# PieSil/CUDA-spectral-ray-tracer

Hardware: AMD Instinct MI355X
Metric: Mray/s (higher is better)
Workload: dtype f32; 1 GPU; random-spheres tri scene (4802 tris, 9603 BVH nodes), 1920x1080, 1024 spp, depth 16; scene_id=100, tiles=8x8 px per wave, rank = tile % n_gpus, gather=none (1 GPU), launch_mode=one process, one GPU

## Files before the change

### cuda-spectral-ray-tracer_amd/csrc/srt_device.h

```cpp
#pragma once
#include <hip/hip_runtime.h>
#include <stdint.h>

#include "srt_color_consts.h"
#include "srt_powf.h"

namespace srt {

constexpr int kCieSamples = 95;
constexpr int kWavelengths = 7;
constexpr float kLambdaMin = 360.0f;
constexpr float kLambdaMax = 830.0f;
constexpr float kEpsilon = 0.0001f;
constexpr float kFltMax = 3.402823466e+38f;

__device__ __noinline__ static float dev_powf(float x, float y) { return srt_powf(x, y); }

struct V3 { float x, y, z; };
__device__ __forceinline__ V3 mk(float x, float y, float z) { V3 r; r.x = x; r.y = y; r.z = z; return r; }
__device__ __forceinline__ V3 operator+(V3 a, V3 b) { return mk(a.x + b.x, a.y + b.y, a.z + b.z); }
__device__ __forceinline__ V3 operator-(V3 a, V3 b) { return mk(a.x - b.x, a.y - b.y, a.z - b.z); }
__device__ __forceinline__ V3 operator-(V3 a) { return mk(-a.x, -a.y, -a.z); }
__device__ __forceinline__ V3 operator*(float t, V3 v) { return mk(t * v.x, t * v.y, t * v.z); }
__device__ __forceinline__ float dot(V3 a, V3 b) { return a.x * b.x + a.y * b.y + a.z * b.z; }
// ... 535 lines not shown
        "v_cmpx_gt_u32 vcc, %[ninner], %[node]\n\t"
        SRT_INNER_VISIT_ASM SRT_INNER_NEXT_ASM
        SRT_INNER_VISIT_ASM SRT_INNER_NEXT_ASM
        SRT_INNER_VISIT_ASM SRT_INNER_NEXT_ASM
        SRT_INNER_VISIT_ASM SRT_INNER_NEXT_ASM
        SRT_INNER_VISIT_ASM SRT_INNER_NEXT_ASM
        SRT_INNER_VISIT_ASM SRT_INNER_NEXT_ASM
        SRT_INNER_VISIT_ASM SRT_INNER_NEXT_ASM
        SRT_INNER_VISIT_ASM
        ".Lsrt_burst_end%=:\n\t"
        "s_mov_b64 exec, s[80:81]\n\t"
        : [node] "+v"(tv.node), [top] "+v"(tv.top), [sp] "+v"(tv.sp)
        : [nf0] "v"(tv.nf[0]), [nf1] "v"(tv.nf[1]), [nf2] "v"(tv.nf[2]), [p0] "v"(p0), [p1] "v"(p1), [p2] "v"(p2), [c] "v"(tv.c),
          [ms] "v"(minus_stride), [ps] "v"(plus_stride), [ninner] "s"(n_inner), [refs] "s"(refs), [stay] "s"(stay)
        : "v100", "v101", "v102", "v103", "v104", "v105", "v106", "v107", "v108", "v109", "v110", "v111", "v112", "v113", "v114",
          "v115", "v116", "v117", "v118", "s80", "s81", "s82", "s83", "s84", "s85", "s86", "vcc", "scc", "memory");
}

#define SRT_INNER_NEXT2_ASM                                                                                              \
    "v_cmpx_gt_u32 vcc, %[ninner], %[node]\n\t"                                                                          \
    "s_bcnt1_i32_b64 s86, exec\n\t"                                                                                      \
    "s_cmp_lt_u32 s86, s87\n\t"                                                                                          \
    "s_cbranch_scc1 .Lsrt_phase_burst_end%=\n\t"
__device__ __forceinline__ uint32_t inner_phase_asm(Trav &tv, const NodeSrc &ns, V3 o, V3 inv, uint32_t n_inner, uint32_t n_alive,
                                                    uint32_t score_shade, uint32_t score_fringe) {
    const f2 p0 = mk2(o.x, o.y), p1 = mk2(o.z, inv.x), p2 = mk2(inv.y, inv.z);
    const int minus_stride = -kStackStride<true>, plus_stride = kStackStride<true>;
    const uint32_t refs = (uint32_t)(uintptr_t)ns.lds_r0;
    uint32_t kind;
    asm volatile(
        "s_mov_b64 s[80:81], exec\n\t"
        ".Lsrt_phase_decide%=:\n\t"
        "v_cmp_lt_i32 vcc, -1, %[node]\n\t"
        "v_cmp_le_i32_e64 s[82:83], %[ninner], %[node]\n\t"
        "s_bcnt1_i32_b64 s86, vcc\n\t"
        "s_bcnt1_i32_b64 s87, s[82:83]\n\t"
        "s_sub_u32 s88, %[nalive], s86\n\t"
        "s_sub_u32 s86, s86, s87\n\t"
        "s_mul_i32 s88, s88, %[wshade]\n\t"
        "s_mul_i32 s89, s87, %[wfringe]\n\t"
        "s_lshl_b32 s84, s86, 8\n\t"
        "s_max_u32 s85, s89, s84\n\t"
        "s_mov_b32 %[kind], 0\n\t"
        "s_cmp_gt_u32 s88, s85\n\t"
        "s_cbranch_scc1 .Lsrt_phase_end%=\n\t"
        "s_mov_b32 %[kind], 1\n\t"
        "s_cmp_gt_u32 s89, s84\n\t"
        "s_cbranch_scc1 .Lsrt_phase_end%=\n\t"
        "s_add_u32 s87, s86, 2\n\t"
        "s_mul_hi_u32 s87, s87, 0xaaaaaaab\n\t"
        "s_lshr_b32 s87, s87, 1\n\t"
        "s_andn2_b64 exec, vcc, s[82:83]\n\t"
        SRT_INNER_VISIT_ASM SRT_INNER_NEXT2_ASM
        SRT_INNER_VISIT_ASM SRT_INNER_NEXT2_ASM
        SRT_INNER_VISIT_ASM SRT_INNER_NEXT2_ASM
        SRT_INNER_VISIT_ASM SRT_INNER_NEXT2_ASM
        SRT_INNER_VISIT_ASM SRT_INNER_NEXT2_ASM
        SRT_INNER_VISIT_ASM SRT_INNER_NEXT2_ASM
        SRT_INNER_VISIT_ASM SRT_INNER_NEXT2_ASM
        SRT_INNER_VISIT_ASM
        ".Lsrt_phase_burst_end%=:\n\t"
        "s_mov_b64 exec, s[80:81]\n\t"
        "s_branch .Lsrt_phase_decide%=\n\t"
        ".Lsrt_phase_end%=:\n\t"
        : [node] "+v"(tv.node), [top] "+v"(tv.top), [sp] "+v"(tv.sp), [kind] "=&s"(kind)
        : [nf0] "v"(tv.nf[0]), [nf1] "v"(tv.nf[1]), [nf2] "v"(tv.nf[2]), [p0] "v"(p0), [p1] "v"(p1), [p2] "v"(p2), [c] "v"(tv.c),
          [ms] "v"(minus_stride), [ps] "v"(plus_stride), [ninner] "s"(n_inner), [refs] "s"(refs), [nalive] "s"(n_alive),
          [wshade] "s"(score_shade), [wfringe] "s"(score_fringe)
        : "v100", "v101", "v102", "v103", "v104", "v105", "v106", "v107", "v108", "v109", "v110", "v111", "v112", "v113", "v114",
          "v115", "v116", "v117", "v118", "s80", "s81", "s82", "s83", "s84", "s85", "s86", "s87", "s88", "s89", "vcc",
          "scc", "memory");
    return kind;
}

#define SRT_INNER_VISIT_MIXED_ASM                                                                                        \
    "ds_write_b32 %[sp], %[top] offset:256\n\t"                                                                          \
    "ds_read_b32 v116, %[sp]\n\t"                                                                              \
    "v_cmp_le_u32 vcc, %[ncached], %[node]\n\t"                                          \
    "s_and_saveexec_b64 s[90:91], vcc\n\t"                                                                               \
    "s_cbranch_execz 1f\n\t"                                                                                             \
    "v_mul_u32_u24 v117, 0x50, %[node]\n\t"                                                          \
    "v_add_u32 v114, v117, %[g0]\n\t"                                                                                    \
    "v_add_u32 v115, v117, %[g1]\n\t"                                                                                    \
    "v_add_u32 v118, v117, %[g2]\n\t"                                                                                    \
    "buffer_load_dwordx4 v[100:103], v114, %[rsrc], 0 offen\n\t"                                                         \
    "buffer_load_dwordx4 v[104:107], v115, %[rsrc], 0 offen offset:24\n\t"                                               \
// ... 61 lines not shown
__device__ __forceinline__ void inner_burst4_mixed_asm(Trav &tv, const NodeSrc &ns, V3 o, V3 inv, uint32_t n_inner, uint32_t stay) {
    const f2 p0 = mk2(o.x, o.y), p1 = mk2(o.z, inv.x), p2 = mk2(inv.y, inv.z);
    const int minus_stride = -kStackStride<false>, plus_stride = kStackStride<false>;
    const uint32_t refs0 = (uint32_t)(uintptr_t)ns.lds_r0, refs1 = (uint32_t)(uintptr_t)ns.lds_r1;
    const uint32_t g0 = tv.nf[0] & 8u, g1 = tv.nf[1] & 8u, g2 = tv.nf[2] & 8u;
    asm volatile(
        "s_mov_b64 s[80:81], exec\n\t"
        "v_cmpx_gt_u32 vcc, %[ninner], %[node]\n\t"
        SRT_INNER_VISIT_MIXED_ASM SRT_INNER_NEXT_MIXED_ASM
        SRT_INNER_VISIT_MIXED_ASM SRT_INNER_NEXT_MIXED_ASM
        SRT_INNER_VISIT_MIXED_ASM SRT_INNER_NEXT_MIXED_ASM
        SRT_INNER_VISIT_MIXED_ASM
        ".Lsrt_mixed_end%=:\n\t"
        "s_mov_b64 exec, s[80:81]\n\t"
        : [node] "+v"(tv.node), [top] "+v"(tv.top), [sp] "+v"(tv.sp)
        : [nf0] "v"(tv.nf[0]), [nf1] "v"(tv.nf[1]), [nf2] "v"(tv.nf[2]), [g0] "v"(g0), [g1] "v"(g1), [g2] "v"(g2), [p0] "v"(p0), [p1] "v"(p1), [p2] "v"(p2),
          [c] "v"(tv.c), [ms] "v"(minus_stride), [ps] "v"(plus_stride), [ninner] "s"(n_inner), [ncached] "s"((uint32_t)ns.n_cached), [refs0] "s"(refs0),
          [refs1] "s"(refs1), [stay] "s"(stay), [rsrc] "s"(ns.global_nodes_sw)
        : "v100", "v101", "v102", "v103", "v104", "v105", "v106", "v107", "v108", "v109", "v110", "v111", "v112", "v113", "v114",
          "v115", "v116", "v117", "v118", "s80", "s81", "s82", "s83", "s84", "s85", "s86", "s90", "s91", "vcc", "scc", "memory");
}

struct FringeFetch { f4v q0, q1, q2, q3, q4, q5; int below; };
template <bool NARROW>
__device__ __forceinline__ void trav_fringe_fetch(FringeFetch &ff, const Trav &tv, const NodeSrc &ns, const StackRef &stack) {
    const uint32_t off = __umul24((uint32_t)(tv.node - ns.n_inner), ns.fringe_stride);
    ff.q0 = buf_load16(ns.global_fringe, off); ff.q1 = buf_load16(ns.global_fringe, off + 16u); ff.q2 = buf_load16(ns.global_fringe, off + 32u);
    ff.q3 = buf_load16(ns.global_fringe, off + 48u); ff.q4 = buf_load16(ns.global_fringe, off + 64u); ff.q5 = buf_load16(ns.global_fringe, off + 80u);
    ff.below = NARROW ? (int)*(lds_i16 *)(uintptr_t)tv.sp : *(lds_i32 *)(uintptr_t)tv.sp;
}
template <bool COUNT, bool NARROW, bool PAIRED = false>
__device__ __forceinline__ void trav_fringe_compute(const FringeFetch &ff, Trav &tv, V3 o, V3 d, V3 inv, float tmin, TravStats &ts) {
    const f4v q0 = ff.q0, q1 = ff.q1, q2 = ff.q2, q3 = ff.q3, q4 = ff.q4, q5 = ff.q5;
    const int below = ff.below;
    const f2 w0 = mk2(q0.x, q0.y), w1 = mk2(q0.z, q0.w), w2 = mk2(q1.x, q1.y), w3 = mk2(q1.z, q1.w), w4 = mk2(q2.x, q2.y), w5 = mk2(q2.z, q2.w);
    const f2 w6 = mk2(q3.x, q3.y), w7 = mk2(q3.z, q3.w), w8 = mk2(q4.x, q4.y), w9 = mk2(q4.z, q4.w);
    const uint32_t fl = __float_as_uint(q5.x), fr = __float_as_uint(q5.y);
    const int lref = (int)__float_as_uint(q5.z), rref = (int)__float_as_uint(q5.w);
    const bool leaf_l = PAIRED || lref < 0, leaf_r = PAIRED || rref < 0;
    if (COUNT) { ts.n_iters++; ts.n_tri += (leaf_l ? 1u : 0u) + (leaf_r ? 1u : 0u); ts.n_box += (leaf_l ? 0u : 1u) + (leaf_r ? 0u : 1u); }

    float e_box = 0.f, m_box = 0.f;
    if (!PAIRED) {
        const bool int_r = !leaf_r;
        const float xlo = int_r ? w0.y : w0.x, xhi = int_r ? w1.y : w1.x, ylo = int_r ? w2.y : w2.x, yhi = int_r ? w3.y : w3.x;
        const float zlo = int_r ? w4.y : w4.x, zhi = int_r ? w5.y : w5.x;
        const bool px = inv.x >= 0, py = inv.y >= 0, pz = inv.z >= 0;
        const float t0x = ((px ? xlo : xhi) - o.x) * inv.x, t1x = ((px ? xhi : xlo) - o.x) * inv.x;
        const float t0y = ((py ? ylo : yhi) - o.y) * inv.y, t1y = ((py ? yhi : ylo) - o.y) * inv.y;
        const float t0z = ((pz ? zlo : zhi) - o.z) * inv.z, t1z = ((pz ? zhi : zlo) - o.z) * inv.z;
        e_box = fmaxf(fmaxf(fmaxf(tmin, t0x), t0y), t0z);
        m_box = fminf(fminf(t1x, t1y), t1z);
    }

    const f2 denom = w0 * d.x + w1 * d.y + w2 * d.z;
    const f2 num = w3 - (w0 * o.x + w1 * o.y + w2 * o.z);
    const f2 t = mk2(num.x / denom.x, num.y / denom.y);
    const bool wyl = fl & kTriWIsY, hzl = fl & kTriHIsZ, wyr = fr & kTriWIsY, hzr = fr & kTriHIsZ;
    const f2 pw = mk2(wyl ? o.y : o.x, wyr ? o.y : o.x) + t * mk2(wyl ? d.y : d.x, wyr ? d.y : d.x);
    const f2 ph = mk2(hzl ? o.z : o.y, hzr ? o.z : o.y) + t * mk2(hzl ? d.z : d.y, hzr ? d.z : d.y);
    const f2 a1 = (pw - w6) * (w5 - w7) - (w4 - w6) * (ph - w7);
    const f2 a2 = (pw - w8) * (w7 - w9) - (w6 - w8) * (ph - w9);
    const f2 a3 = (pw - w4) * (w9 - w5) - (w8 - w4) * (ph - w5);
    const uint32_t sl = fl & 0x80000000u, sr = fr & 0x80000000u;
    float m_l = inside_min2(a1.x, a2.x, sl);
    float m_r = inside_min2(a1.y, a2.y, sr);
    asm volatile("" : "+v"(m_l), "+v"(m_r));
    const bool in_l = inside_min3(m_l, a3.x, sl);
    const bool in_r = inside_min3(m_r, a3.y, sr);
    const bool ok_l = leaf_l & !(fabsf(denom.x) < 1e-8f) & (tmin <= t.x) & in_l;
    const bool ok_r = leaf_r & !(fabsf(denom.y) < 1e-8f) & (tmin <= t.y) & in_r;

    const float c0 = tv.c;
    const bool hit_l = ok_l & (t.x <= c0);
    const float c1 = hit_l ? t.x : c0;
    const bool hit_r = ok_r & (t.y <= c1);
    const float c2 = hit_r ? t.y : c1;
    tv.c = c2;
    tv.hit = hit_r ? ~rref : (hit_l ? ~lref : tv.hit);
    const int top = tv.top;
    if (PAIRED) {
        tv.node = top;
        tv.top = below;
        tv.sp += (uint32_t)(-kStackStride<NARROW>);
        return;
    }
    const bool pass = !(fminf(leaf_r ? c0 : c1, m_box) <= e_box);
    const bool go = !(leaf_l & leaf_r) & pass;
    tv.node = go ? (leaf_r ? lref : rref) : top;
    tv.top = go ? top : below;
    tv.sp += (uint32_t)(go ? 0 : -kStackStride<NARROW>);
}
template <bool COUNT, bool NARROW, bool PAIRED = false>
__device__ __forceinline__ void trav_step_fringe(Trav &tv, const NodeSrc &ns, V3 o, V3 d, V3 inv, float tmin, const StackRef &stack, TravStats &ts) {
    FringeFetch ff;
    trav_fringe_fetch<NARROW>(ff, tv, ns, stack);
    trav_fringe_compute<COUNT, NARROW, PAIRED>(ff, tv, o, d, inv, tmin, ts);
}


}
```

### cuda-spectral-ray-tracer_amd/csrc/srt_kernels.hip

```cpp
#include <algorithm>
#include <stdlib.h>

#include "srt_color_consts.h"
#include "srt_kernel_common.h"

namespace srt {

#ifndef SRT_INNER_BURST
#define SRT_INNER_BURST 8
#endif
#ifndef SRT_BURST_DROP
#define SRT_BURST_DROP 3
#endif
#ifndef SRT_ASM_BURST
#define SRT_ASM_BURST 2
#endif
#ifndef SRT_INNER_BURST_L2
#define SRT_INNER_BURST_L2 4
#endif
#ifndef SRT_ASM_BURST_L2
#define SRT_ASM_BURST_L2 1
#endif
#ifndef SRT_BURST_DROP_L2
#define SRT_BURST_DROP_L2 2
// ... 26 lines not shown
}
void render_launch_plan(int stack_depth, int n_records, int n_inner, const PlanKnobs &k, LaunchPlan &lp) {
    render_launch_shape(stack_depth, n_records, n_inner, k, lp.waves_per_block, lp.n_cached);
    lp.all_cached = lp.n_cached == n_inner;
    lp.waves_per_eu = 4;
    lp.blocks_per_cu = 16 / lp.waves_per_block;
    lp.waves_per_cu = lp.waves_per_block * lp.blocks_per_cu;
}
RenderGrid render_launch_grid(const LaunchPlan &lp, uint32_t n_cu, uint32_t waves_per_cu_override, uint32_t queue_rows_bound) {
    RenderGrid g;
    g.waves_per_block = lp.waves_per_block;
    uint32_t waves_per_cu = (uint32_t)lp.waves_per_cu;
    if (waves_per_cu_override > 0 && waves_per_cu_override < 16 && g.waves_per_block == 16) {
        g.waves_per_block = (int)waves_per_cu_override;
        waves_per_cu = waves_per_cu_override;
    }
    uint32_t n_waves = n_cu * waves_per_cu;
    if (n_waves > queue_rows_bound) n_waves = queue_rows_bound;
    g.n_blocks = (n_waves + (uint32_t)g.waves_per_block - 1) / (uint32_t)g.waves_per_block;
    g.waves = g.n_blocks * (uint32_t)g.waves_per_block;
    return g;
}

#ifndef SRT_PAIRED_VARIANT
#define SRT_PAIRED_VARIANT 1
#endif
bool render_paired_variant(bool tree_is_paired, bool narrow, bool all_cached) { return SRT_PAIRED_VARIANT != 0 && tree_is_paired && narrow == all_cached; }

#ifndef SRT_ASSIGN_PERM
#define SRT_ASSIGN_PERM 0
#endif
__device__ __forceinline__ uint32_t assigned_band(uint32_t w) {
    if (SRT_ASSIGN_PERM == 1) return (w & 3u) * 4u + (w >> 2);
    if (SRT_ASSIGN_PERM == 2) return (w & 4u) ? ((w & ~3u) | (3u - (w & 3u))) : w;
    return w;
}

__global__ void init_rng_kernel(uint32_t *rng, uint32_t n_lanes, uint64_t seed) {
    uint32_t idx = blockIdx.x * blockDim.x + threadIdx.x;
    if (idx >= n_lanes) return;
    Rng s;
    rng_seed(s, seed + idx);
    rng[0 * (size_t)n_lanes + idx] = s.d;
    rng[1 * (size_t)n_lanes + idx] = s.v0;
    rng[2 * (size_t)n_lanes + idx] = s.v1;
    rng[3 * (size_t)n_lanes + idx] = s.v2;
// ... 100 lines not shown
    ns.lds_r0 = (lds_cu32 *)s_r0; ns.lds_r1 = (lds_cu32 *)s_r1;
    ns.n_cached = P.n_cached;
    const buf_rsrc shade_rsrc = make_rsrc(P.shade, P.n_tris * 48u);
    const buf_rsrc sd_rsrc = make_rsrc(P.mat_sd, (P.n_materials + 1u) * 768u);
    const uint32_t spp = P.spp;
    uint32_t w_shade = P.score_shade, w_fringe = P.score_fringe;
    asm volatile("" : "+s"(w_shade), "+s"(w_fringe));
    StackRef my_stack;
    {
        const size_t slots = (size_t)(P.stack_depth < 1 ? 1 : P.stack_depth) + kStackSentinels;
        my_stack.s16 = (lds_i16 *)(s_stack_base + (size_t)wave * slots * 128u) + lane;
        my_stack.s32 = (lds_i32 *)(s_stack_base + (size_t)wave * slots * 256u) + lane;
        stack_init<NARROW>(my_stack);
    }

    bool dead = false, have_path = false, have_pixel = false;
    uint32_t idx = 0;
    uint32_t out_slot = 0;
    uint32_t pixel_ij = 0;
    Rng rs; rs.d = rs.v0 = rs.v1 = rs.v2 = rs.v3 = rs.v4 = 0u;
    V3 acc = mk(0.f, 0.f, 0.f);
    float acc2 = 0.f;
    uint32_t sample = 0, bounce = 0, valid = 0;
    V3 ro = mk(0.f, 0.f, 0.f), rd = mk(0.f, 0.f, 1.f), inv = mk(0.f, 0.f, 1.f);
    float hero = kLambdaMin;
    float pw[kWavelengths];
#pragma unroll
    for (int k = 0; k < kWavelengths; k++) pw[k] = 0.f;
    Trav tv; tv.node = kTravIdle; tv.sp = 0u; tv.top = -1; tv.c = kFltMax; tv.hit = -1; tv.nf[0] = tv.nf[1] = tv.nf[2] = 0u;
    uint32_t n_rays = 0;
    TravStats ts;
    bool parked = false, exclusive = false;
    OrderProfile prof;
    prof.magic = 0; prof.seg = nullptr;
    if (COUNT && P.wave_debug) prof = *reinterpret_cast<const OrderProfile *>(P.wave_debug);
    unsigned long long t_shade = 0, t_inner = 0, t_fringe = 0, t_mark = 0;
    if (COUNT) t_mark = __builtin_amdgcn_s_memtime();
    const unsigned long long t_born = t_mark;
    unsigned long long t_dry = 0;
    uint32_t cur_tile_local = 0, pixel_iters0 = 0;
    uint32_t pixel_rays0 = 0, max_pix_iters = 0, max_pix_rays = 0;
    uint32_t w_shade_passes = 0, l_shade = 0, l_cam = 0, w_reject_iters = 0;
    uint32_t n_hits = 0;

    for (;;) {
        if (__ballot(have_pixel) == 0ull) parked = false;
        if (__ballot(!dead && !parked && tv.node < 0) != 0ull) {
            bool end_path = false, begin_trav = false;
            if (COUNT) { w_shade_passes++; l_shade += (uint32_t)__popcll(__ballot(!dead && tv.node == kTravDone)); }
            float xyz_x = 0.0f, xyz_y = 0.0f, xyz_z = 0.0f;

            if (!dead && tv.node == kTravDone) {
                tv.node = kTravIdle;
                if (COUNT && P.wave_debug && prof.seg != nullptr) {
                    const bool walked = !(rd.x != rd.x || rd.y != rd.y || rd.z != rd.z);
                    const unsigned long long m = __ballot(walked);
                    if (walked) {
                        const int leader = __ffsll((long long)m) - 1;
                        uint32_t base = 0;
                        if ((int)lane == leader) base = atomicAdd(prof.seg_tickets, (uint32_t)__popcll(m));
                        base = (uint32_t)__shfl((int)base, leader, 64);
                        const uint32_t ticket = base + (uint32_t)__popcll(m & ((1ull << lane) - 1ull));
                        const uint32_t key = ticket + prof.seg_phase;
                        const uint32_t slot = key / prof.seg_stride - (prof.seg_phase ? 1u : 0u);
                        if (key % prof.seg_stride == 0u && (unsigned long long)slot < prof.seg_capacity) {
                            const float t_end = tv.hit < 0 ? kFltMax : tv.c;
                            prof.seg[2 * (size_t)slot] = make_float4(ro.x, ro.y, ro.z, rd.x);
                            prof.seg[2 * (size_t)slot + 1] = make_float4(rd.y, rd.z, t_end, __int_as_float(tv.hit));
                        }
                    }
                }
                float wl[kWavelengths];
                hero_expand(hero, wl);
                uint32_t sd_table = P.n_materials;
                bool was_hit = false, hit_scattered = false;
                if (tv.hit < 0) {
                    end_path = true;
                } else {
                    if (COUNT && P.wave_debug && prof.magic == kOrderProfileMagic) {
                        int k = prof.leaf[tv.hit];
                        for (int guard = 0; guard < 96; guard++) {
                            const int up = prof.up[k];
                            if (up < 0) break;
                            const float *b = prof.sibbox + 6 * (size_t)k;
                            const float x0 = (b[0] - ro.x) * inv.x, x1 = (b[1] - ro.x) * inv.x;
                            const float y0 = (b[2] - ro.y) * inv.y, y1 = (b[3] - ro.y) * inv.y;
                            const float z0 = (b[4] - ro.z) * inv.z, z1 = (b[5] - ro.z) * inv.z;
                            const float e = fmaxf(fmaxf(fmaxf(0.0f, fminf(x0, x1)), fminf(y0, y1)), fminf(z0, z1));
                            const float m = fminf(fminf(fmaxf(x0, x1), fmaxf(y0, y1)), fmaxf(z0, z1));
                            if (e <= m && e > tv.c) atomicAdd(&prof.cnt[up], 1u);
                            k = up >> 1;
                        }
                    }
                    const uint32_t srec = __umul24((uint32_t)tv.hit, 48u);
                    const f4v s0 = buf_load16(shade_rsrc, srec), s1 = buf_load16(shade_rsrc, srec + 16u), s2 = buf_load16(shade_rsrc, srec + 32u);
                    const V3 n_geo = mk(s0.x, s0.y, s0.z);
                    const V3 hp = ro + tv.c * rd;
                    const bool front_face = dot(rd, n_geo) < 0;
                    const V3 n = front_face ? n_geo : -n_geo;
                    const uint32_t mat = __float_as_uint(s0.w);
                    const uint32_t mtype = __float_as_uint(s1.x);
                    const float fuzz = s1.y;

                    V3 scatter_direction = mk(0.f, 0.f, 0.f);
                    float eps_sign = 1.0f;
                    bool did_scatter = true;
                    const V3 unit_in = unit_vector(rd);
                    if (mtype == 4u) {
                        did_scatter = false;
                    } else if (mtype == 2u) {
                        float ir = sellmeier_index(s1.z, s1.w, s2.x, s2.y, s2.z, s2.w, wl[0]);
                        float refraction_ratio = front_face ? (1.0f / ir) : ir;
                        float cos_theta = fminf(dot(-unit_in, n), 1.0f);
                        float sin_theta = sqrtf(1.0f - cos_theta * cos_theta);
                        bool cannot_refract = refraction_ratio * sin_theta > 1.0f;
                        if (!cannot_refract)
                            cannot_refract = reflectance(cos_theta, refraction_ratio) > rng_uniform(rs);
                        if (cannot_refract) {
                            scatter_direction = reflect(unit_in, n);
                        } else {
                            scatter_direction = refract(unit_in, n, refraction_ratio);
                            eps_sign = -1.0f;
                            valid = 1;
                        }
                    } else {
                        const V3 ruv = random_unit_vector(rs);
                        if (mtype == 1u) {
                            V3 reflected = reflect(unit_in, n);
                            scatter_direction = reflected + fuzz * ruv;
                            did_scatter = dot(scatter_direction, n) > 0;
// ... 1 lines not shown
                        } else {
                            scatter_direction = n + ruv;
                            if (near_zero(scatter_direction)) scatter_direction = n;
                        }
                    }
                    if constexpr (FEATURES) {
                        if (bounce == 0u) {
                            const uint32_t rows_lo = (uint32_t)__builtin_amdgcn_readfirstlane((int)((FILM && !ADAPT) ? U->accum_sum2[0] : U->accum_film[0])), rows_hi = (uint32_t)__builtin_amdgcn_readfirstlane((int)((FILM && !ADAPT) ? U->accum_sum2[1] : U->accum_film[1]));
                            const uint32_t col_lo = (uint32_t)__builtin_amdgcn_readfirstlane((int)((ADAPT || FILM) ? U->tile_cost[0] : U->accum_sum2[0])), col_hi = (uint32_t)__builtin_amdgcn_readfirstlane((int)((ADAPT || FILM) ? U->tile_cost[1] : U->accum_sum2[1]));
                            float4 *row = join_ptr<float4>(rows_lo, rows_hi) + (size_t)idx * (kFeatureStride / 4u);
                            if constexpr (FILM && ADAPT) row += (size_t)U->n_lanes * (kFilmStride / 4u);
                            const buf_rsrc col_rsrc = make_rsrc(join_ptr<const float>(col_lo, col_hi), P.n_materials * 16u);
                            const uint32_t col_off = (mat < P.n_materials ? mat : P.n_materials) * 16u;
                            {
                                float4 f = row[0];
                                const float red = __uint_as_float(__builtin_amdgcn_raw_buffer_load_b32(col_rsrc, (int)col_off, 0, 0));
                                f.x = f.x + n.x; f.y = f.y + n.y; f.z = f.z + n.z; f.w = f.w + red;
                                row[0] = f;
                            }
                            asm volatile("" ::: "memory");
                            {
                                float4 f = row[1];
                                const float2 gb = buf_load8(col_rsrc, col_off + 4u);
                                const float dist = tv.c * sqrtf((rd.x * rd.x + rd.y * rd.y) + rd.z * rd.z);
                                f.x = f.x + gb.x; f.y = f.y + gb.y; f.z = f.z + dist; f.w = f.w + 1.0f;
                                row[1] = f;
                            }
                        }
                    }
                    sd_table = mat;
                    ro = hp + (eps_sign * kEpsilon) * n;
                    rd = scatter_direction;
                    hit_scattered = did_scatter;
                    was_hit = true;
                    if (COUNT) n_hits++;
                }
                const bool ends_here = !was_hit || !hit_scattered;
                const float delta_lambda = (kLambdaMax - kLambdaMin) / (float)kWavelengths;
                const uint32_t sd_base = __umul24(sd_table, 768u);
                int off[kWavelengths];
                float wgt[kWavelengths];
                float2 sp[kWavelengths];
#pragma unroll
                for (int k = 0; k < kWavelengths; k++) {
                    interp_coords(wl[k], off[k], wgt[k]);
                    sp[k] = buf_load8(sd_rsrc, sd_base + (uint32_t)off[k] * 8u);
                }
#pragma unroll
                for (int k = 0; k < kWavelengths; k++) pw[k] *= interp_pair(sp[k], wgt[k]);
                if (ends_here) {
#pragma unroll
                    for (int k = 0; k < kWavelengths; k++) {
                        const float4 r0 = s_cmf[off[k]], r1 = s_cmf[off[k] + 1];
                        const float w = wgt[k], power = (uint32_t)k < valid ? pw[k] : 0.0f;
                        xyz_x += ((1.0f - w) * r0.x + w * r1.x) * power * delta_lambda;
// ... 204 lines not shown
            if (COUNT) l_cam += (uint32_t)__popcll(__ballot(!dead && tv.node < 0 && !have_path && !begin_trav && have_pixel && sample < spp));
            if (!dead && tv.node < 0 && !have_path && !begin_trav && have_pixel && sample < spp) {
                float px = -0.5f + rng_uniform(rs);
                float py = -0.5f + rng_uniform(rs);
                const V3 du = mk(U->du[0], U->du[1], U->du[2]), dv = mk(U->dv[0], U->dv[1], U->dv[2]);
                const V3 cam_center = mk(U->center[0], U->center[1], U->center[2]);
                const V3 pixel_center = (mk(U->p00[0], U->p00[1], U->p00[2]) + (float)(U->offx + (pixel_ij & 0xffffu)) * du) + (float)(U->offy + (pixel_ij >> 16)) * dv;
                V3 pixel_sample = pixel_center + (px * du + py * dv);
                V3 origin = cam_center;
                if (!(U->defocus_angle <= 0.0f)) {
                    float dx, dy;
#if SRT_ASM_RNG
                    rng_disk_loop_asm(rs, dx, dy);
#else
                    for (;;) {
                        dx = rng_pm1(rs);
                        dy = rng_pm1(rs);
                        if ((dx * dx + dy * dy) + 0.0f * 0.0f < 1.0f) break;
                    }
#endif
                    origin = (cam_center + dx * mk(U->disk_u[0], U->disk_u[1], U->disk_u[2])) +
                             dy * mk(U->disk_v[0], U->disk_v[1], U->disk_v[2]);
                }
                ro = origin;
                rd = pixel_sample - origin;
                hero = hero_draw(rs);
#pragma unroll
                for (int k = 0; k < kWavelengths; k++) pw[k] = 1.0f;
                valid = kWavelengths;
                sample++;
                bounce = 0;
                have_path = true;
                if (P.bounce_limit > 0) begin_trav = true;
                else { valid = 0;
                       have_path = false;  }
            }

            if (begin_trav) {
                n_rays++;
                inv = mk(1.0f / rd.x, 1.0f / rd.y, 1.0f / rd.z);
                ray_near_addresses(ns, inv, tv.nf);
                (void)trav_begin<ITERS>(tv, stack_base<NARROW>(my_stack), P.tris, P.root_ref, ro, rd, 0.0f, kFltMax, ts);
            }
        }

        if (COUNT) { const unsigned long long now = __builtin_amdgcn_s_memtime(); t_shade += now - t_mark; t_mark = now; }
        if (__ballot(!dead) == 0ull) break;
        const unsigned long long alive_mask = __ballot(!dead && !parked);
        if (alive_mask == 0ull) continue;
        const uint32_t n_alive = (uint32_t)__popcll(alive_mask);
        const uint32_t n_inner_u = (uint32_t)P.n_inner;
        if (!COUNT && n_alive == 1u) {
            while (__ballot(tv.node >= 0) != 0ull) {
                if (tv.node >= 0) {
                    if ((uint32_t)tv.node < n_inner_u) trav_step_inner<ITERS, NARROW, ALL_CACHED>(tv, ns, ro, inv, 0.0f, my_stack, ts);
                    else trav_step_fringe<ITERS, NARROW, PAIRED>(tv, ns, ro, rd, inv, 0.0f, my_stack, ts);
                }
            }
            continue;
        }
        if (!ITERS && NARROW && ALL_CACHED && kInnerBurst == 8 && kBurstDrop == 3u && SRT_ASM_BURST == 2) {
            while (inner_phase_asm(tv, ns, ro, inv, n_inner_u, n_alive, w_shade, w_fringe) != 0u) {
                if (tv.node >= (int)n_inner_u) trav_step_fringe<ITERS, NARROW, PAIRED>(tv, ns, ro, rd, inv, 0.0f, my_stack, ts);
            }
        } else
        for (;;) {
            const unsigned long long trav_mask = __ballot(tv.node >= 0);
            if (trav_mask == 0ull) break;
            const unsigned long long fringe_mask = __ballot(tv.node >= (int)n_inner_u);
            const uint32_t n_trav = (uint32_t)__popcll(trav_mask), n_fringe = (uint32_t)__popcll(fringe_mask);
            const uint32_t s_sh = (n_alive - n_trav) * P.score_shade;
            const uint32_t s_fr = n_fringe * P.score_fringe;
            const uint32_t s_in = (n_trav - n_fringe) << 8;
            if (s_sh > max(s_fr, s_in)) break;
            const bool do_fringe = s_fr > s_in;
            if (COUNT) { ts.w_iters++; ts.w_alive += n_alive; if (do_fringe) { ts.w_fringe++; ts.l_fringe += n_fringe; } else ts.l_inner += n_trav - n_fringe; }
            if (do_fringe) {
                if (tv.node >= (int)n_inner_u) trav_step_fringe<ITERS, NARROW, PAIRED>(tv, ns, ro, rd, inv, 0.0f, my_stack, ts);
                if (COUNT) { const unsigned long long now = __builtin_amdgcn_s_memtime(); t_fringe += now - t_mark; t_mark = now; }
            } else {
                bool at_inner = (uint32_t)tv.node < n_inner_u;
                constexpr int burst_len = ALL_CACHED ? kInnerBurst : kInnerBurstL2;
                constexpr uint32_t burst_drop = ALL_CACHED ? kBurstDrop : kBurstDropL2;
                const uint32_t stay = (n_trav - n_fringe + burst_drop - 1u) / burst_drop;
                if (!ITERS && NARROW && ALL_CACHED && kInnerBurst == 8 && SRT_ASM_BURST == 1) {
                    inner_burst8_asm(tv, ns, ro, inv, n_inner_u, stay);
                } else if (!ITERS && !NARROW && !ALL_CACHED && kInnerBurstL2 == 4 && SRT_ASM_BURST_L2 && P.nodes_sw != nullptr) {
                    inner_burst4_mixed_asm(tv, ns, ro, inv, n_inner_u, stay);
                } else
#pragma unroll
                for (int burst = 0; burst < burst_len; burst++) {
                    if (at_inner) trav_step_inner<ITERS, NARROW, ALL_CACHED>(tv, ns, ro, inv, 0.0f, my_stack, ts);
                    at_inner = (uint32_t)tv.node < n_inner_u;
                    const unsigned long long m = __ballot(at_inner);
                    if (COUNT && burst > 0) { ts.w_iters++; ts.w_alive += n_alive; }
                    if (COUNT && burst < burst_len - 1) ts.l_inner += (uint32_t)__popcll(m);
                    if ((uint32_t)__popcll(m) < stay) break;
                }
                if (COUNT) { const unsigned long long now = __builtin_amdgcn_s_memtime(); t_inner += now - t_mark; t_mark = now; }
            }
        }
    }

    {
        uint32_t r = wave_sum(n_rays);
        if (!PROBE && lane == 0 && r) atomicAdd(&P.counters[0], (unsigned long long)r);
        if (COUNT) {
            uint32_t a = wave_sum(ts.n_iters), b = wave_sum(ts.n_tri), c = wave_sum(ts.n_box);
            if (lane == 0) {
                atomicAdd(&P.counters[1], (unsigned long long)a);
                atomicAdd(&P.counters[2], (unsigned long long)b);
                atomicAdd(&P.counters[3], (unsigned long long)c);
                atomicAdd(&P.counters[4], (unsigned long long)ts.w_iters);
                atomicAdd(&P.counters[5], (unsigned long long)ts.w_alive);
            }
// ... 480 lines not shown
```

Measured before the change: 16590 Mray/s.

## Pop stack inside asm phase loop and visit fringe with packed ray registers

When the fringe phase is chosen, the inner-phase asm now records the fringe node, pops the traversal stack itself, and returns. The fringe leaf is then fetched and intersected from the recorded index, without a separate stack read or pop afterward. Ray origin, direction and inverse are kept in packed f2 register pairs so the triangle plane dot products can use v_pk_mul_f32 with broadcast operands. An option also runs the fringe visit on all lanes without a per-lane check. This aims to shorten the dependency chain between phases and cut register shuffling, at the cost of extra register layout complexity and possible wasted loads on non-fringe lanes.

```diff
diff --git a/cuda-spectral-ray-tracer_amd/csrc/srt_device.h b/cuda-spectral-ray-tracer_amd/csrc/srt_device.h
--- a/cuda-spectral-ray-tracer_amd/csrc/srt_device.h
+++ b/cuda-spectral-ray-tracer_amd/csrc/srt_device.h
@@ -581,6 +581,99 @@
     "s_bcnt1_i32_b64 s86, exec\n\t"                                                                                      \
     "s_cmp_lt_u32 s86, s87\n\t"                                                                                          \
     "s_cbranch_scc1 .Lsrt_phase_burst_end%=\n\t"
+template <bool PAIRS> struct RayRegs;
+template <> struct RayRegs<false> {
+    V3 o, d, i;
+    __device__ __forceinline__ V3 ro() const { return o; }
+    __device__ __forceinline__ V3 rd() const { return d; }
+    __device__ __forceinline__ V3 inv() const { return i; }
+    __device__ __forceinline__ void set_ro(V3 v) { o = v; }
+    __device__ __forceinline__ void set_rd(V3 v) { d = v; }
+    __device__ __forceinline__ void set_inv(V3 v) { i = v; }
+    __device__ __forceinline__ f2 p0() const { return mk2(o.x, o.y); }
+    __device__ __forceinline__ f2 p1() const { return mk2(o.z, i.x); }
+    __device__ __forceinline__ f2 p2() const { return mk2(i.y, i.z); }
+};
+template <> struct RayRegs<true> {
+    f2 q0, q1, q2, d0, d1;
+    __device__ __forceinline__ V3 ro() const { return mk(q0.x, q0.y, q1.x); }
+    __device__ __forceinline__ V3 rd() const { return mk(d0.x, d0.y, d1.x); }
+    __device__ __forceinline__ V3 inv() const { return mk(q1.y, q2.x, q2.y); }
+    __device__ __forceinline__ void set_ro(V3 v) { q0.x = v.x; q0.y = v.y; q1.x = v.z; }
+    __device__ __forceinline__ void set_rd(V3 v) { d0.x = v.x; d0.y = v.y; d1.x = v.z; d1.y = v.z; }
+    __device__ __forceinline__ void set_inv(V3 v) { q1.y = v.x; q2.x = v.y; q2.y = v.z; }
+    __device__ __forceinline__ f2 p0() const { return q0; }
+    __device__ __forceinline__ f2 p1() const { return q1; }
+    __device__ __forceinline__ f2 p2() const { return q2; }
+};
+template <int HALF>
+__device__ __forceinline__ f2 pk_bcast_mul(f2 p, f2 w) {
+    f2 r;
+    if (HALF == 0) asm("v_pk_mul_f32 %0, %1, %2 op_sel_hi:[0,1]" : "=v"(r) : "v"(p), "v"(w));
+    else asm("v_pk_mul_f32 %0, %1, %2 op_sel:[1,0]" : "=v"(r) : "v"(p), "v"(w));
+    return r;
+}
+
+#define SRT_PHASE_DECIDE_ASM(FRINGE_LABEL, ENTRY)                                                                         \
+        "s_mov_b64 s[80:81], exec\n\t"                                                                                   \
+        ENTRY                                                                                                            \
+        ".Lsrt_phase_decide%=:\n\t"                                                                                      \
+        "v_cmp_lt_i32 vcc, -1, %[node]\n\t"                                                              \
+        "v_cmp_le_i32_e64 s[82:83], %[ninner], %[node]\n\t"                                  \
+        "s_bcnt1_i32_b64 s86, vcc\n\t"                                                                                   \
+        "s_bcnt1_i32_b64 s87, s[82:83]\n\t"                                                                              \
+        "s_sub_u32 s88, %[nalive], s86\n\t"                                        \
+        "s_sub_u32 s86, s86, s87\n\t"                                                      \
+        "s_mul_i32 s88, s88, %[wshade]\n\t"                                                                              \
+        "s_mul_i32 s89, s87, %[wfringe]\n\t"                                                                             \
+        "s_lshl_b32 s84, s86, 8\n\t"                                                                                     \
+        "s_max_u32 s85, s89, s84\n\t"                                                                                    \
+        "s_mov_b32 %[kind], 0\n\t"                                                                                       \
+        "s_cmp_gt_u32 s88, s85\n\t"                                                                                      \
+        "s_cbranch_scc1 .Lsrt_phase_end%=\n\t"                                 \
+        "s_mov_b32 %[kind], 1\n\t"                                                                                       \
+        "s_cmp_gt_u32 s89, s84\n\t"                                                                                      \
+        "s_cbranch_scc1 " FRINGE_LABEL "%=\n\t"                                                        \
+        "s_add_u32 s87, s86, 2\n\t"                                                    \
+        "s_mul_hi_u32 s87, s87, 0xaaaaaaab\n\t"                                                                          \
+        "s_lshr_b32 s87, s87, 1\n\t"                                                                                     \
+        "s_andn2_b64 exec, vcc, s[82:83]\n\t"                                            \
+        SRT_INNER_VISIT_ASM SRT_INNER_NEXT2_ASM                                                                          \
+        SRT_INNER_VISIT_ASM SRT_INNER_NEXT2_ASM                                                                          \
+        SRT_INNER_VISIT_ASM SRT_INNER_NEXT2_ASM                                                                          \
+        SRT_INNER_VISIT_ASM SRT_INNER_NEXT2_ASM                                                                          \
+        SRT_INNER_VISIT_ASM SRT_INNER_NEXT2_ASM                                                                          \
+        SRT_INNER_VISIT_ASM SRT_INNER_NEXT2_ASM                                                                          \
+        SRT_INNER_VISIT_ASM SRT_INNER_NEXT2_ASM                                                                          \
+        SRT_INNER_VISIT_ASM                                                                                              \
+        ".Lsrt_phase_burst_end%=:\n\t"                                                                                   \
+        "s_mov_b64 exec, s[80:81]\n\t"                                                                                   \
+        "s_branch .Lsrt_phase_decide%=\n\t"
+__device__ __forceinline__ uint32_t inner_phase_pop_asm(Trav &tv, int &rec, const NodeSrc &ns, f2 p0, f2 p1, f2 p2, uint32_t n_inner, uint32_t n_alive,
+                                                        uint32_t score_shade, uint32_t score_fringe) {
+    const int minus_stride = -kStackStride<true>, plus_stride = kStackStride<true>;
+    const uint32_t refs = (uint32_t)(uintptr_t)ns.lds_r0;
+    uint32_t kind;
+    asm volatile(
+        SRT_PHASE_DECIDE_ASM(".Lsrt_phase_fringe", "")
+        ".Lsrt_phase_fringe%=:\n\t"
+        "v_mov_b32 %[rec], %[node]\n\t"
+        "s_mov_b64 exec, s[82:83]\n\t"
+        "v_mov_b32 %[node], %[top]\n\t"
+        "ds_read_i16 %[top], %[sp]\n\t"
+        "v_add_u32 %[sp], %[ms], %[sp]\n\t"
+        "s_mov_b64 exec, s[80:81]\n\t"
+        "s_waitcnt lgkmcnt(0)\n\t"
+        ".Lsrt_phase_end%=:\n\t"
+        : [node] "+v"(tv.node), [top] "+v"(tv.top), [sp] "+v"(tv.sp), [kind] "=&s"(kind), [rec] "=&v"(rec)
+        : [nf0] "v"(tv.nf[0]), [nf1] "v"(tv.nf[1]), [nf2] "v"(tv.nf[2]), [p0] "v"(p0), [p1] "v"(p1), [p2] "v"(p2), [c] "v"(tv.c),
+          [ms] "v"(minus_stride), [ps] "v"(plus_stride), [ninner] "s"(n_inner), [refs] "s"(refs), [nalive] "s"(n_alive),
+          [wshade] "s"(score_shade), [wfringe] "s"(score_fringe)
+        : "v100", "v101", "v102", "v103", "v104", "v105", "v106", "v107", "v108", "v109", "v110", "v111", "v112", "v113", "v114",
+          "v115", "v116", "v117", "v118", "s80", "s81", "s82", "s83", "s84", "s85", "s86", "s87", "s88", "s89", "vcc",
+          "scc", "memory");
+    return kind;
+}
 __device__ __forceinline__ uint32_t inner_phase_asm(Trav &tv, const NodeSrc &ns, V3 o, V3 inv, uint32_t n_inner, uint32_t n_alive,
                                                     uint32_t score_shade, uint32_t score_fringe) {
     const f2 p0 = mk2(o.x, o.y), p1 = mk2(o.z, inv.x), p2 = mk2(inv.y, inv.z);
@@ -588,39 +681,7 @@
     const uint32_t refs = (uint32_t)(uintptr_t)ns.lds_r0;
     uint32_t kind;
     asm volatile(
-        "s_mov_b64 s[80:81], exec\n\t"
-        ".Lsrt_phase_decide%=:\n\t"
-        "v_cmp_lt_i32 vcc, -1, %[node]\n\t"
-        "v_cmp_le_i32_e64 s[82:83], %[ninner], %[node]\n\t"
-        "s_bcnt1_i32_b64 s86, vcc\n\t"
-        "s_bcnt1_i32_b64 s87, s[82:83]\n\t"
-        "s_sub_u32 s88, %[nalive], s86\n\t"
-        "s_sub_u32 s86, s86, s87\n\t"
-        "s_mul_i32 s88, s88, %[wshade]\n\t"
-        "s_mul_i32 s89, s87, %[wfringe]\n\t"
-        "s_lshl_b32 s84, s86, 8\n\t"
-        "s_max_u32 s85, s89, s84\n\t"
-        "s_mov_b32 %[kind], 0\n\t"
-        "s_cmp_gt_u32 s88, s85\n\t"
-        "s_cbranch_scc1 .Lsrt_phase_end%=\n\t"
-        "s_mov_b32 %[kind], 1\n\t"
-        "s_cmp_gt_u32 s89, s84\n\t"
-        "s_cbranch_scc1 .Lsrt_phase_end%=\n\t"
-        "s_add_u32 s87, s86, 2\n\t"
-        "s_mul_hi_u32 s87, s87, 0xaaaaaaab\n\t"
-        "s_lshr_b32 s87, s87, 1\n\t"
-        "s_andn2_b64 exec, vcc, s[82:83]\n\t"
-        SRT_INNER_VISIT_ASM SRT_INNER_NEXT2_ASM
-        SRT_INNER_VISIT_ASM SRT_INNER_NEXT2_ASM
-        SRT_INNER_VISIT_ASM SRT_INNER_NEXT2_ASM
-        SRT_INNER_VISIT_ASM SRT_INNER_NEXT2_ASM
-        SRT_INNER_VISIT_ASM SRT_INNER_NEXT2_ASM
-        SRT_INNER_VISIT_ASM SRT_INNER_NEXT2_ASM
-        SRT_INNER_VISIT_ASM SRT_INNER_NEXT2_ASM
-        SRT_INNER_VISIT_ASM
-        ".Lsrt_phase_burst_end%=:\n\t"
-        "s_mov_b64 exec, s[80:81]\n\t"
-        "s_branch .Lsrt_phase_decide%=\n\t"
+        SRT_PHASE_DECIDE_ASM(".Lsrt_phase_end", "")
         ".Lsrt_phase_end%=:\n\t"
         : [node] "+v"(tv.node), [top] "+v"(tv.top), [sp] "+v"(tv.sp), [kind] "=&s"(kind)
         : [nf0] "v"(tv.nf[0]), [nf1] "v"(tv.nf[1]), [nf2] "v"(tv.nf[2]), [p0] "v"(p0), [p1] "v"(p1), [p2] "v"(p2), [c] "v"(tv.c),
@@ -728,15 +789,20 @@
 }
 
 struct FringeFetch { f4v q0, q1, q2, q3, q4, q5; int below; };
+__device__ __forceinline__ void trav_fringe_fetch_record(FringeFetch &ff, int node, const NodeSrc &ns) {
+    const uint32_t off = __umul24((uint32_t)(node - ns.n_inner), ns.fringe_stride);
+    ff.q0 = buf_load16(ns.global_fringe, off); ff.q1 = buf_load16(ns.global_fringe, off + 16u); ff.q2 = buf_load16(ns.global_fringe, off + 32u);
+    ff.q3 = buf_load16(ns.global_fringe, off + 48u); ff.q4 = buf_load16(ns.global_fringe, off + 64u); ff.q5 = buf_load16(ns.global_fringe, off + 80u);
+}
 template <bool NARROW>
 __device__ __forceinline__ void trav_fringe_fetch(FringeFetch &ff, const Trav &tv, const NodeSrc &ns, const StackRef &stack) {
-    const uint32_t off = __umul24((uint32_t)(tv.node - ns.n_inner), ns.fringe_stride);
-    ff.q0 = buf_load16(ns.global_fringe, off); ff.q1 = buf_load16(ns.global_fringe, off + 16u); ff.q2 = buf_load16(ns.global_fringe, off + 32u);
-    ff.q3 = buf_load16(ns.global_fringe, off + 48u); ff.q4 = buf_load16(ns.global_fringe, off + 64u); ff.q5 = buf_load16(ns.global_fringe, off + 80u);
+    trav_fringe_fetch_record(ff, tv.node, ns);
     ff.below = NARROW ? (int)*(lds_i16 *)(uintptr_t)tv.sp : *(lds_i32 *)(uintptr_t)tv.sp;
 }
-template <bool COUNT, bool NARROW, bool PAIRED = false>
-__device__ __forceinline__ void trav_fringe_compute(const FringeFetch &ff, Trav &tv, V3 o, V3 d, V3 inv, float tmin, TravStats &ts) {
+template <bool COUNT, bool NARROW, bool PAIRED = false, bool POP = true>
+__device__ __forceinline__ void trav_fringe_compute(const FringeFetch &ff, Trav &tv, V3 o, V3 d, V3 inv, float tmin, TravStats &ts,
+                                                    const RayRegs<true> *bc = nullptr) {
+    static_assert(POP || PAIRED, "only the PAIRED visit always pops");
     const f4v q0 = ff.q0, q1 = ff.q1, q2 = ff.q2, q3 = ff.q3, q4 = ff.q4, q5 = ff.q5;
     const int below = ff.below;
     const f2 w0 = mk2(q0.x, q0.y), w1 = mk2(q0.z, q0.w), w2 = mk2(q1.x, q1.y), w3 = mk2(q1.z, q1.w), w4 = mk2(q2.x, q2.y), w5 = mk2(q2.z, q2.w);
@@ -759,8 +825,15 @@
         m_box = fminf(fminf(t1x, t1y), t1z);
     }
 
-    const f2 denom = w0 * d.x + w1 * d.y + w2 * d.z;
-    const f2 num = w3 - (w0 * o.x + w1 * o.y + w2 * o.z);
+    f2 denom, n_o;
+    if (bc) {
+        denom = pk_bcast_mul<0>(bc->d0, w0) + pk_bcast_mul<1>(bc->d0, w1) + pk_bcast_mul<0>(bc->d1, w2);
+        n_o = pk_bcast_mul<0>(bc->q0, w0) + pk_bcast_mul<1>(bc->q0, w1) + pk_bcast_mul<0>(bc->q1, w2);
+    } else {
+        denom = w0 * d.x + w1 * d.y + w2 * d.z;
+        n_o = w0 * o.x + w1 * o.y + w2 * o.z;
+    }
+    const f2 num = w3 - n_o;
     const f2 t = mk2(num.x / denom.x, num.y / denom.y);
     const bool wyl = fl & kTriWIsY, hzl = fl & kTriHIsZ, wyr = fr & kTriWIsY, hzr = fr & kTriHIsZ;
     const f2 pw = mk2(wyl ? o.y : o.x, wyr ? o.y : o.x) + t * mk2(wyl ? d.y : d.x, wyr ? d.y : d.x);
@@ -784,6 +857,7 @@
     const float c2 = hit_r ? t.y : c1;
     tv.c = c2;
     tv.hit = hit_r ? ~rref : (hit_l ? ~lref : tv.hit);
+    if (PAIRED && !POP) return;
     const int top = tv.top;
     if (PAIRED) {
         tv.node = top;
@@ -803,6 +877,15 @@
     trav_fringe_fetch<NARROW>(ff, tv, ns, stack);
     trav_fringe_compute<COUNT, NARROW, PAIRED>(ff, tv, o, d, inv, tmin, ts);
 }
-
-
-}
+__device__ __forceinline__ const RayRegs<true> *bcast_pairs(const RayRegs<true> &ray) { return &ray; }
+__device__ __forceinline__ const RayRegs<true> *bcast_pairs(const RayRegs<false> &) { return nullptr; }
+template <bool PAIRS>
+__device__ __forceinline__ void trav_visit_fringe_popped(Trav &tv, int rec, const NodeSrc &ns, const RayRegs<PAIRS> &ray, TravStats &ts) {
+    FringeFetch ff;
+    trav_fringe_fetch_record(ff, rec, ns);
+    ff.below = 0;
+    trav_fringe_compute<false, true, true, false>(ff, tv, ray.ro(), ray.rd(), ray.inv(), 0.0f, ts, bcast_pairs(ray));
+}
+
+
+}
diff --git a/cuda-spectral-ray-tracer_amd/csrc/srt_kernels.hip b/cuda-spectral-ray-tracer_amd/csrc/srt_kernels.hip
--- a/cuda-spectral-ray-tracer_amd/csrc/srt_kernels.hip
+++ b/cuda-spectral-ray-tracer_amd/csrc/srt_kernels.hip
@@ -72,6 +72,15 @@
     return g;
 }
 
+#ifndef SRT_GLUE_POP
+#define SRT_GLUE_POP 1
+#endif
+#ifndef SRT_GLUE_PAIRS
+#define SRT_GLUE_PAIRS 1
+#endif
+#ifndef SRT_GLUE_ALL_LANES
+#define SRT_GLUE_ALL_LANES 1
+#endif
 #ifndef SRT_PAIRED_VARIANT
 #define SRT_PAIRED_VARIANT 1
 #endif
@@ -218,7 +227,9 @@
     V3 acc = mk(0.f, 0.f, 0.f);
     float acc2 = 0.f;
     uint32_t sample = 0, bounce = 0, valid = 0;
-    V3 ro = mk(0.f, 0.f, 0.f), rd = mk(0.f, 0.f, 1.f), inv = mk(0.f, 0.f, 1.f);
+    constexpr bool RAY_PAIRS = SRT_GLUE_PAIRS && !ITERS && NARROW && ALL_CACHED && PAIRED;
+    RayRegs<RAY_PAIRS> ray;
+    ray.set_ro(mk(0.f, 0.f, 0.f)); ray.set_rd(mk(0.f, 0.f, 1.f)); ray.set_inv(mk(0.f, 0.f, 1.f));
     float hero = kLambdaMin;
     float pw[kWavelengths];
 #pragma unroll
@@ -249,7 +260,7 @@
             if (!dead && tv.node == kTravDone) {
                 tv.node = kTravIdle;
                 if (COUNT && P.wave_debug && prof.seg != nullptr) {
-                    const bool walked = !(rd.x != rd.x || rd.y != rd.y || rd.z != rd.z);
+                    const bool walked = !(ray.rd().x != ray.rd().x || ray.rd().y != ray.rd().y || ray.rd().z != ray.rd().z);
                     const unsigned long long m = __ballot(walked);
                     if (walked) {
                         const int leader = __ffsll((long long)m) - 1;
@@ -261,8 +272,8 @@
                         const uint32_t slot = key / prof.seg_stride - (prof.seg_phase ? 1u : 0u);
                         if (key % prof.seg_stride == 0u && (unsigned long long)slot < prof.seg_capacity) {
                             const float t_end = tv.hit < 0 ? kFltMax : tv.c;
-                            prof.seg[2 * (size_t)slot] = make_float4(ro.x, ro.y, ro.z, rd.x);
-                            prof.seg[2 * (size_t)slot + 1] = make_float4(rd.y, rd.z, t_end, __int_as_float(tv.hit));
+                            prof.seg[2 * (size_t)slot] = make_float4(ray.ro().x, ray.ro().y, ray.ro().z, ray.rd().x);
+                            prof.seg[2 * (size_t)slot + 1] = make_float4(ray.rd().y, ray.rd().z, t_end, __int_as_float(tv.hit));
                         }
                     }
                 }
@@ -279,9 +290,9 @@
                             const int up = prof.up[k];
                             if (up < 0) break;
                             const float *b = prof.sibbox + 6 * (size_t)k;
-                            const float x0 = (b[0] - ro.x) * inv.x, x1 = (b[1] - ro.x) * inv.x;
-                            const float y0 = (b[2] - ro.y) * inv.y, y1 = (b[3] - ro.y) * inv.y;
-                            const float z0 = (b[4] - ro.z) * inv.z, z1 = (b[5] - ro.z) * inv.z;
+                            const float x0 = (b[0] - ray.ro().x) * ray.inv().x, x1 = (b[1] - ray.ro().x) * ray.inv().x;
+                            const float y0 = (b[2] - ray.ro().y) * ray.inv().y, y1 = (b[3] - ray.ro().y) * ray.inv().y;
+                            const float z0 = (b[4] - ray.ro().z) * ray.inv().z, z1 = (b[5] - ray.ro().z) * ray.inv().z;
                             const float e = fmaxf(fmaxf(fmaxf(0.0f, fminf(x0, x1)), fminf(y0, y1)), fminf(z0, z1));
                             const float m = fminf(fminf(fmaxf(x0, x1), fmaxf(y0, y1)), fmaxf(z0, z1));
                             if (e <= m && e > tv.c) atomicAdd(&prof.cnt[up], 1u);
@@ -291,8 +302,8 @@
                     const uint32_t srec = __umul24((uint32_t)tv.hit, 48u);
                     const f4v s0 = buf_load16(shade_rsrc, srec), s1 = buf_load16(shade_rsrc, srec + 16u), s2 = buf_load16(shade_rsrc, srec + 32u);
                     const V3 n_geo = mk(s0.x, s0.y, s0.z);
-                    const V3 hp = ro + tv.c * rd;
-                    const bool front_face = dot(rd, n_geo) < 0;
+                    const V3 hp = ray.ro() + tv.c * ray.rd();
+                    const bool front_face = dot(ray.rd(), n_geo) < 0;
                     const V3 n = front_face ? n_geo : -n_geo;
                     const uint32_t mat = __float_as_uint(s0.w);
                     const uint32_t mtype = __float_as_uint(s1.x);
@@ -301,7 +312,7 @@
                     V3 scatter_direction = mk(0.f, 0.f, 0.f);
                     float eps_sign = 1.0f;
                     bool did_scatter = true;
-                    const V3 unit_in = unit_vector(rd);
+                    const V3 unit_in = unit_vector(ray.rd());
                     if (mtype == 4u) {
                         did_scatter = false;
                     } else if (mtype == 2u) {
@@ -349,15 +360,15 @@
                             {
                                 float4 f = row[1];
                                 const float2 gb = buf_load8(col_rsrc, col_off + 4u);
-                                const float dist = tv.c * sqrtf((rd.x * rd.x + rd.y * rd.y) + rd.z * rd.z);
+                                const float dist = tv.c * sqrtf((ray.rd().x * ray.rd().x + ray.rd().y * ray.rd().y) + ray.rd().z * ray.rd().z);
                                 f.x = f.x + gb.x; f.y = f.y + gb.y; f.z = f.z + dist; f.w = f.w + 1.0f;
                                 row[1] = f;
                             }
                         }
                     }
                     sd_table = mat;
-                    ro = hp + (eps_sign * kEpsilon) * n;
-                    rd = scatter_direction;
+                    ray.set_ro(hp + (eps_sign * kEpsilon) * n);
+                    ray.set_rd(scatter_direction);
                     hit_scattered = did_scatter;
                     was_hit = true;
                     if (COUNT) n_hits++;
@@ -608,8 +619,8 @@
                     origin = (cam_center + dx * mk(U->disk_u[0], U->disk_u[1], U->disk_u[2])) +
                              dy * mk(U->disk_v[0], U->disk_v[1], U->disk_v[2]);
                 }
-                ro = origin;
-                rd = pixel_sample - origin;
+                ray.set_ro(origin);
+                ray.set_rd(pixel_sample - origin);
                 hero = hero_draw(rs);
 #pragma unroll
                 for (int k = 0; k < kWavelengths; k++) pw[k] = 1.0f;
@@ -624,9 +635,9 @@
 
             if (begin_trav) {
                 n_rays++;
-                inv = mk(1.0f / rd.x, 1.0f / rd.y, 1.0f / rd.z);
-                ray_near_addresses(ns, inv, tv.nf);
-                (void)trav_begin<ITERS>(tv, stack_base<NARROW>(my_stack), P.tris, P.root_ref, ro, rd, 0.0f, kFltMax, ts);
+                ray.set_inv(mk(1.0f / ray.rd().x, 1.0f / ray.rd().y, 1.0f / ray.rd().z));
+                ray_near_addresses(ns, ray.inv(), tv.nf);
+                (void)trav_begin<ITERS>(tv, stack_base<NARROW>(my_stack), P.tris, P.root_ref, ray.ro(), ray.rd(), 0.0f, kFltMax, ts);
             }
         }
 
@@ -639,15 +650,21 @@
         if (!COUNT && n_alive == 1u) {
             while (__ballot(tv.node >= 0) != 0ull) {
                 if (tv.node >= 0) {
-                    if ((uint32_t)tv.node < n_inner_u) trav_step_inner<ITERS, NARROW, ALL_CACHED>(tv, ns, ro, inv, 0.0f, my_stack, ts);
-                    else trav_step_fringe<ITERS, NARROW, PAIRED>(tv, ns, ro, rd, inv, 0.0f, my_stack, ts);
+                    if ((uint32_t)tv.node < n_inner_u) trav_step_inner<ITERS, NARROW, ALL_CACHED>(tv, ns, ray.ro(), ray.inv(), 0.0f, my_stack, ts);
+                    else trav_step_fringe<ITERS, NARROW, PAIRED>(tv, ns, ray.ro(), ray.rd(), ray.inv(), 0.0f, my_stack, ts);
                 }
             }
             continue;
         }
         if (!ITERS && NARROW && ALL_CACHED && kInnerBurst == 8 && kBurstDrop == 3u && SRT_ASM_BURST == 2) {
-            while (inner_phase_asm(tv, ns, ro, inv, n_inner_u, n_alive, w_shade, w_fringe) != 0u) {
-                if (tv.node >= (int)n_inner_u) trav_step_fringe<ITERS, NARROW, PAIRED>(tv, ns, ro, rd, inv, 0.0f, my_stack, ts);
+            if (PAIRED && SRT_GLUE_POP) {
+                int rec;
+                while (inner_phase_pop_asm(tv, rec, ns, ray.p0(), ray.p1(), ray.p2(), n_inner_u, n_alive, w_shade, w_fringe) != 0u) {
+                    if (SRT_GLUE_ALL_LANES || rec >= (int)n_inner_u) trav_visit_fringe_popped(tv, rec, ns, ray, ts);
+                }
+            } else
+            while (inner_phase_asm(tv, ns, ray.ro(), ray.inv(), n_inner_u, n_alive, w_shade, w_fringe) != 0u) {
+                if (tv.node >= (int)n_inner_u) trav_step_fringe<ITERS, NARROW, PAIRED>(tv, ns, ray.ro(), ray.rd(), ray.inv(), 0.0f, my_stack, ts);
             }
         } else
         for (;;) {
@@ -662,7 +679,7 @@
             const bool do_fringe = s_fr > s_in;
             if (COUNT) { ts.w_iters++; ts.w_alive += n_alive; if (do_fringe) { ts.w_fringe++; ts.l_fringe += n_fringe; } else ts.l_inner += n_trav - n_fringe; }
             if (do_fringe) {
-                if (tv.node >= (int)n_inner_u) trav_step_fringe<ITERS, NARROW, PAIRED>(tv, ns, ro, rd, inv, 0.0f, my_stack, ts);
+                if (tv.node >= (int)n_inner_u) trav_step_fringe<ITERS, NARROW, PAIRED>(tv, ns, ray.ro(), ray.rd(), ray.inv(), 0.0f, my_stack, ts);
                 if (COUNT) { const unsigned long long now = __builtin_amdgcn_s_memtime(); t_fringe += now - t_mark; t_mark = now; }
             } else {
                 bool at_inner = (uint32_t)tv.node < n_inner_u;
@@ -670,13 +687,13 @@
                 constexpr uint32_t burst_drop = ALL_CACHED ? kBurstDrop : kBurstDropL2;
                 const uint32_t stay = (n_trav - n_fringe + burst_drop - 1u) / burst_drop;
                 if (!ITERS && NARROW && ALL_CACHED && kInnerBurst == 8 && SRT_ASM_BURST == 1) {
-                    inner_burst8_asm(tv, ns, ro, inv, n_inner_u, stay);
+                    inner_burst8_asm(tv, ns, ray.ro(), ray.inv(), n_inner_u, stay);
                 } else if (!ITERS && !NARROW && !ALL_CACHED && kInnerBurstL2 == 4 && SRT_ASM_BURST_L2 && P.nodes_sw != nullptr) {
-                    inner_burst4_mixed_asm(tv, ns, ro, inv, n_inner_u, stay);
+                    inner_burst4_mixed_asm(tv, ns, ray.ro(), ray.inv(), n_inner_u, stay);
                 } else
 #pragma unroll
                 for (int burst = 0; burst < burst_len; burst++) {
-                    if (at_inner) trav_step_inner<ITERS, NARROW, ALL_CACHED>(tv, ns, ro, inv, 0.0f, my_stack, ts);
+                    if (at_inner) trav_step_inner<ITERS, NARROW, ALL_CACHED>(tv, ns, ray.ro(), ray.inv(), 0.0f, my_stack, ts);
                     at_inner = (uint32_t)tv.node < n_inner_u;
                     const unsigned long long m = __ballot(at_inner);
                     if (COUNT && burst > 0) { ts.w_iters++; ts.w_alive += n_alive; }
```

Result: no change. 16710 Mray/s (median of 6 runs) (+0.8%).
